# ashvardanian/StringZilla

Measured on AMD Instinct MI355X. Metric: DP cell-updates/s (GCUPS) on 1M-pair Levenshtein batch, higher is better.
Workload: dtype u32 bit-vectors (u64 results)

## Files before the change

### stringzilla_amd/csrc/hip/kernels.h

```cpp
#ifndef SZS_ROCM_KERNELS_H_
#define SZS_ROCM_KERNELS_H_

#include <stddef.h>
#include <stdint.h>

#ifdef __cplusplus
extern "C" {
#endif

typedef struct szs_string_ref_t {
    uint64_t address;
    uint32_t length;
    uint32_t index;
} szs_string_ref_t;

#define SZS_LAYOUT_SYMMETRIC 1
#define SZS_LAYOUT_TRANSPOSED 2

#define SZS_CANDIDATES_PER_WORKGROUP 256u
#define SZS_MYERS_MAX_WORDS 64u
#define SZS_MYERS_SHORT_WORDS 8u

unsigned szs_hip_levenshtein_myers_round_words(unsigned words);

// ... 171 lines not shown
    szs_knob_split_k,
    szs_knob_alphabet_k,
    szs_knob_merge_k,
    szs_knob_team_k,
    szs_knob_queues_k,
    szs_knob_roctx_k,
    szs_knob_queue_k,
    szs_knob_queue_words_k,
    szs_knob_queue_rounds_k,
    szs_knob_queue_priority_k,
    szs_knob_fused_k,
    szs_knob_tiny_k,
    szs_knob_top_k_tile_k,
    szs_knob_rerank_k,
    szs_knob_fuzzy_search_segment_k,
    szs_knob_fuzzy_scan_piece_k,
    szs_knob_count_k
};
int szs_tuning_get(int knob);


#define SZS_PLAN_VARIANTS 10u
#define SZS_PLAN_DEVICE_LONGEST 6143u
#define SZS_PLAN_STATUS_DESCENDING 1u
#define SZS_PLAN_STATUS_OVERFLOW 2u
#define SZS_PLAN_STATUS_UNSORTED 4u

typedef struct szs_side_stats_t {
    uint32_t count, longest;
    uint64_t symbols;
    uint64_t bands_systolic;
    uint64_t bands_chain;
} szs_side_stats_t;

typedef struct szs_plan_side_t {
    void const *offsets;
    uint64_t base;
    uint32_t count, wide;
    szs_string_ref_t *ascending, *descending;
    uint32_t const *lengths;
    uint64_t const *starts;
} szs_plan_side_t;

typedef struct szs_plan_expectation_t {
    uint32_t enabled;
    uint32_t query_side;
    uint32_t longest[2];
    uint32_t variant_counts[SZS_PLAN_VARIANTS];
    uint32_t sequence;
    uint64_t const *runes_needed;
    uint64_t runes_capacity;
    uint32_t const *alphabet_flags;
    uint32_t alphabet;
} szs_plan_expectation_t;

#define SZS_PLAN_RANK_SAMPLES 32u
typedef struct szs_plan_summary_t {
    uint32_t status;
    uint32_t speculation_held;
    szs_side_stats_t side[2];
    uint32_t variant_counts[2][SZS_PLAN_VARIANTS];
    uint64_t symmetric_cells;
    uint32_t sequence;
    uint32_t rank_lengths[2][SZS_PLAN_RANK_SAMPLES + 1];
} szs_plan_summary_t;
#define SZS_PLAN_TIMESTAMPS_AT 448u

int szs_hip_plan(szs_plan_side_t const *queries, szs_plan_side_t const *candidates, unsigned myers_words,
                 szs_plan_expectation_t const *expected, szs_plan_summary_t *summary,
                 uint32_t *verdicts ,
                 void *stream);

#define SZS_FUSED_MOST_STRINGS 1024u
#define SZS_FUSED_MOST_STRINGS_TWO_PASSES 16384u
#define SZS_FUSED_BINS 1024u
typedef struct szs_fused_side_report_t {
    uint32_t sequence;
    uint32_t status;
    uint32_t blank;
    uint32_t pairing;
    szs_side_stats_t stats;
    uint32_t rank_lengths[SZS_PLAN_RANK_SAMPLES + 1];
    uint32_t ticks[5];
    uint32_t padding;
    uint64_t squares;
} szs_fused_side_report_t;
typedef struct szs_fused_plan_t {
    szs_plan_side_t side[2];
    uint32_t sequence;
    uint32_t *ready;
    szs_fused_side_report_t *report;
    uint32_t *gave_up;
    uint32_t poll_budget;
    uint32_t withhold;
    uint32_t symmetric;
    uint32_t blocks_per_group;
} szs_fused_plan_t;
#define SZS_FUSED_POLL_BUDGET (1u << 18)
int szs_hip_levenshtein_myers_fused(szs_fused_plan_t const *plan, uint64_t *results, uint64_t results_row_stride, int layout,
                                    void *stream);

int szs_hip_utf8_transcode(szs_string_ref_t const *strings, uint32_t count, uint64_t const *rune_starts, uint32_t *runes,
                           uint32_t *rune_counts, uint32_t *any_multibyte, void *stream);

int szs_hip_utf8_transcode_tape(void const *data, void const *offsets, uint32_t count, int wide, void const *before_offsets,
                                uint32_t before_count, int before_wide, uint64_t capacity, uint32_t *runes, uint64_t *rune_starts,
                                uint32_t *rune_counts, uint32_t *any_multibyte, uint64_t *needed, void *alphabet_workspace, void *stream);
int szs_hip_utf8_transcode_tapes(void const *first_data, void const *first_offsets, uint32_t first_count, int first_wide,
                                 void const *second_data, void const *second_offsets, uint32_t second_count, int second_wide,
                                 uint64_t capacity, uint32_t *runes, uint64_t *rune_starts, uint32_t *rune_counts,
                                 uint32_t *any_multibyte, uint64_t *needed, void *alphabet_workspace, void *stream);

#define SZS_ALPHABET_SLOTS (1u << 16)
#define SZS_ALPHABET_MOST 4095u
#define SZS_ALPHABET_WORTH_BYTES (1u << 16)
int szs_hip_alphabet_rename(uint32_t count, uint64_t const *rune_starts, uint32_t const *rune_counts, uint32_t *runes,
                            uint32_t const *any_multibyte, void *workspace, int workspace_is_empty, uint32_t most, uint32_t *alphabet_out,
                            void *stream);
size_t szs_hip_alphabet_workspace_bytes(void);

typedef struct szs_cost_model_t {
    int16_t substitution[32 * 32];
    uint8_t byte_to_class[256];
    int32_t gap_open;
    int32_t gap_extend;
    int32_t uniform_match, uniform_mismatch;
} szs_cost_model_t;

enum {
    szs_objective_global_k = 0,
    szs_objective_local_k = 1,
    szs_objective_distance_k = 2,
    szs_objective_distance_runes_k = 3,
    szs_objective_local_saturating_k = 4
};

int szs_hip_weighted_scores(int objective, int affine, int narrow, szs_cost_model_t const *model, szs_string_ref_t const *queries,
                            uint32_t queries_count, szs_string_ref_t const *candidates, uint32_t candidates_count,
                            uint32_t longest_candidate, int64_t *results, uint64_t results_row_stride, int symmetric,
                            void *boundary, void *stream);
size_t szs_hip_weighted_boundary_bytes(int objective, int affine, int narrow, uint32_t queries_count, uint32_t candidates_count,
                                       uint32_t longest_candidate);

int szs_hip_weighted_packed_scores(int local, int affine, uint32_t classes, szs_cost_model_t const *model,
                                   szs_string_ref_t const *queries, uint32_t queries_count, szs_string_ref_t const *candidates,
                                   uint32_t candidates_count, uint32_t longest_candidate, int64_t *results,
                                   uint64_t results_row_stride, int symmetric, void *boundary, void *stream);
size_t szs_hip_weighted_packed_boundary_bytes(int local, int affine, uint32_t classes, uint32_t queries_count,
                                              uint32_t candidates_count, uint32_t longest_candidate);

unsigned szs_hip_weighted_team_shape(unsigned index);
int szs_hip_weighted_team_has_shape(unsigned shape);
uint32_t szs_hip_weighted_team_reach_limit(int objective, int wide);
int szs_hip_weighted_team_fits(unsigned shape, uint32_t classes);
unsigned szs_hip_weighted_team_candidates_per_item(unsigned shape);
int szs_hip_byte_presence(void const *data, void const *offsets, uint32_t count, int wide, uint32_t *presence, void *stream);
int szs_hip_weighted_team_scores(int objective, int affine, int wide, unsigned shape, uint32_t classes, szs_cost_model_t const *model,
                                 szs_string_ref_t const *queries, uint32_t queries_count, szs_string_ref_t const *candidates,
                                 uint32_t candidates_count, uint32_t longest_candidate, int64_t *results,
                                 uint64_t results_row_stride, int symmetric, void *workspace, void *stream);
size_t szs_hip_weighted_team_workspace_bytes(int objective, int affine, int wide, unsigned shape, uint32_t classes, uint32_t queries_count,
                                             uint32_t candidates_count, uint32_t longest_candidate);

int szs_hip_wide_scores(int objective, int affine, szs_cost_model_t const *model, szs_string_ref_t const *queries,
                        uint32_t queries_count, szs_string_ref_t const *candidates, uint32_t candidates_count,
                        uint32_t longest_query, uint32_t longest_candidate, int64_t *results, uint64_t results_row_stride,
                        int layout, void *workspace, void *stream);
// ... 37 lines not shown
```

### stringzilla_amd/csrc/hip/lev_myers.hip

```cpp
#include "myers_core.hpp"

#define SZS_PAIR_RULE_FN __host__ __device__ static inline
#include "pair_rule.h"

#include <cstdlib>

namespace szs_hip {

#ifndef SZS_MYERS_PACK_QUERIES
#define SZS_MYERS_PACK_QUERIES 1
#endif
#ifndef SZS_MYERS_PAIR_RULES
#define SZS_MYERS_PAIR_RULES 1
#endif

#ifndef SZS_MYERS_SHORT_TEXT_DWORDS
#define SZS_MYERS_SHORT_TEXT_DWORDS 2
#endif


__device__ __forceinline__ u32 bits_in_word(u32 from, u32 to, int w) {
    u32 const low = from > 32u * w ? from : 32u * w, high = to < 32u * w + 32u ? to : 32u * w + 32u;
    if (low >= high) return 0u;
    return (high - low == 32u ? ~0u : (1u << (high - low)) - 1u) << (low - 32u * w);
}

template <int words_, int text_dwords_, bool runes_, bool paired_ = false>
__device__ __forceinline__ void myers_workgroup(u32 *peq, u32 *keys, szs_string_ref_t const query,
                                                szs_string_ref_t const *__restrict__ candidates, u32 candidates_count,
                                                u32 candidate_block, u64 *__restrict__ results, u64 results_row_stride,
                                                int symmetric, szs_ref_guard_t const &guard, u32 alphabet = 0,
                                                u32 *claimed_rows = nullptr, u32 blocks_here = 1, szs_string_ref_t const second = {}) {
    static_assert(!paired_ || !runes_, "query pairs are a byte-kernel shape");
    constexpr int rows = runes_ ? rune_slots_k : byte_rows_k;
    using layout = peq_layout<words_, rows>;
    if (guard.enabled && (!ref_is_current(guard, 0, query) || (paired_ && !ref_is_current(guard, 0, second)))) {
        if (threadIdx.x == 0) *guard.stale = guard.sequence;
        return;
    }
    u32 const first_length = query.length, second_length = paired_ ? second.length : 0u;
    u32 const query_length = paired_ ? first_length + second_length : first_length;
    u32 const used_rows = paired_ ? query_length + 2u : query_length;
    u32 const pad = 32u * words_ - used_rows;
    u32 const second_row = pad + first_length + 2u;

    for (int i = threadIdx.x; i < layout::total_dwords; i += 256) peq[i] = 0;
    if constexpr (runes_) {
        if (alphabet) {
            for (u32 i = threadIdx.x; i <= alphabet; i += 256) keys[i] = 0;
            if (threadIdx.x == 0) *claimed_rows = 0;
        }
        else
            for (int i = threadIdx.x; i < rune_slots_k; i += 256) keys[i] = rune_slot_empty_k;
    }
    __syncthreads();
    if (runes_ && alphabet) {
        u32 const *pattern = reinterpret_cast<u32 const *>(query.address);
        for (u32 i = threadIdx.x; i < query_length; i += 256) {
            u32 const id = pattern[i];
            if (atomicCAS(&keys[id], 0u, ~0u) == 0u) keys[id] = atomicAdd(claimed_rows, 1u) + 1;
        }
        __syncthreads();
        for (u32 i = threadIdx.x; i < query_length; i += 256) {
            u32 const position = pad + i;
            atomicOr(&peq[layout::dword_index((int)keys[pattern[i]], (int)(position >> 5))], 1u << (position & 31));
        }
    }
    else if constexpr (runes_) {
        u32 const *pattern = reinterpret_cast<u32 const *>(query.address);
        for (u32 i = threadIdx.x; i < query_length; i += 256) {
            u32 const rune = pattern[i];
            u32 slot = rune_slot_hash(rune);
            for (;;) {
                u32 const previous = atomicCAS(&keys[slot], rune_slot_empty_k, rune);
                if (previous == rune_slot_empty_k || previous == rune) break;
                slot = (slot + 1) & (rune_slots_k - 1);
            }
            u32 const position = pad + i;
            atomicOr(&peq[layout::dword_index((int)slot, (int)(position >> 5))], 1u << (position & 31));
        }
    }
    else {
        u8 const *pattern = reinterpret_cast<u8 const *>(query.address);
        for (u32 i = threadIdx.x; i < first_length; i += 256) {
            u32 const position = pad + i;
            atomicOr(&peq[layout::dword_index(pattern[i], (int)(position >> 5))], 1u << (position & 31));
        }
        if constexpr (paired_) {
            u8 const *above = reinterpret_cast<u8 const *>(second.address);
            for (u32 i = threadIdx.x; i < second_length; i += 256) {
                u32 const position = second_row + i;
                atomicOr(&peq[layout::dword_index(above[i], (int)(position >> 5))], 1u << (position & 31));
            }
        }
    }
    __syncthreads();
    pattern_pair_t<words_> boundary;
    if constexpr (paired_) {
#pragma unroll
        for (int w = 0; w < words_; ++w) {
            boundary.separators[w] = bits_in_word(second_row - 2u, second_row, w);
            boundary.tops[w] = first_length ? bits_in_word(second_row - 3u, second_row - 2u, w) : 0u;
        }
    }

#pragma unroll 1
    for (u32 block_step = 0; block_step < blocks_here; ++block_step) {
    u32 const candidate_slot = (candidate_block - block_step) * SZS_CANDIDATES_PER_WORKGROUP + threadIdx.x;
    bool live = candidate_slot < candidates_count;
    szs_string_ref_t candidate = {0, 0, 0};
    if (live) candidate = candidates[candidate_slot];
    if (live && guard.enabled && !ref_is_current(guard, 1, candidate)) {
        *guard.stale = guard.sequence;
        live = false;
    }
    if ((symmetric & SZS_LAYOUT_SYMMETRIC) && candidate.index > query.index) live = false;
    u32 const text_length = live ? candidate.length : 0;
    u32 const longest_in_wave = wave_max_u32(text_length);
    u32 const shortest_in_wave = ~wave_max_u32(live ? ~text_length : 0u);

    u32 vp[words_], vn[words_];
#pragma unroll
    for (int w = 0; w < words_; ++w) {
        vp[w] = bits_in_word(pad, 32u * words_, w) & ~(paired_ ? boundary.separators[w] : 0u);
        vn[w] = 0;
    }

    auto take = [&](u32 symbol) {
        u32 eq[words_];
        load_match_masks<words_, rows>(peq, !runes_ ? symbol : alphabet ? keys[symbol] : find_rune_slot(keys, symbol), eq);
        if constexpr (paired_) myers_column<words_>(vp, vn, eq, boundary);
        else myers_column<words_>(vp, vn, eq);
    };

    u32 column = 0;
    if constexpr (runes_) {
        u32 const *const runes = reinterpret_cast<u32 const *>(candidate.address);
        auto quad_at = [&](u32 index) -> uint4 {
            return index < text_length ? *reinterpret_cast<uint4 const *>(runes + index) : make_uint4(0, 0, 0, 0);
        };
        if (4 <= shortest_in_wave && longest_in_wave) {
            uint4 ahead = quad_at(0);
            for (; column + 4 <= shortest_in_wave; column += 4) {
                uint4 const now = ahead;
                ahead = quad_at(column + 4);
                take(now.x), take(now.y), take(now.z), take(now.w);
            }
        }
#pragma unroll 1
        for (; column < longest_in_wave; ++column)
            if (column < text_length) take(runes[column]);
    }
    else {
        u64 const safe_address = text_length ? candidate.address : first_length || !paired_ ? query.address : second.address;
        text_stream_t text(safe_address, text_length);
        if (!text_length) text.valid_dwords = query_length ? 1 : 0;
        u32 raw_low = text.raw(0);
        u32 dword = 0;
        constexpr u32 columns_per_iteration = 4 * text_dwords_;
#ifndef SZS_MYERS_CLAMPED_READS
#define SZS_MYERS_CLAMPED_READS(TEXT_DWORDS) ((TEXT_DWORDS) == 1)
#endif
        constexpr bool clamped_reads = SZS_MYERS_CLAMPED_READS(text_dwords_);
        if (columns_per_iteration <= shortest_in_wave && longest_in_wave && query_length) {
            u32 ahead[text_dwords_];
#pragma unroll
            for (int d = 0; d < text_dwords_; ++d) ahead[d] = clamped_reads ? text.raw_clamped(1 + d) : text.raw(1 + d);
            for (; column + columns_per_iteration <= shortest_in_wave;
                 column += columns_per_iteration, dword += text_dwords_) {
                u32 symbols[text_dwords_];
                symbols[0] = text.splice(raw_low, ahead[0]);
#pragma unroll
                for (int d = 1; d < text_dwords_; ++d) symbols[d] = text.splice(ahead[d - 1], ahead[d]);
                raw_low = ahead[text_dwords_ - 1];
#pragma unroll
                for (int d = 0; d < text_dwords_; ++d)
                    ahead[d] = clamped_reads ? text.raw_clamped(dword + text_dwords_ + 1 + d)
                                             : text.raw(dword + text_dwords_ + 1 + d);
#pragma unroll
                for (int step = 0; step < 4 * text_dwords_; ++step) take((symbols[step / 4] >> (8 * (step % 4))) & 0xFFu);
            }
        }
#ifndef SZS_MYERS_MID_LOOP
#define SZS_MYERS_MID_LOOP 0
#endif
        if constexpr (SZS_MYERS_MID_LOOP && text_dwords_ > 1) {
            if (column + 4 <= shortest_in_wave && longest_in_wave && query_length) {
                u32 ahead_one = text.raw(dword + 1);
#pragma unroll 1
                for (; column + 4 <= shortest_in_wave; column += 4, ++dword) {
                    u32 const symbols = text.splice(raw_low, ahead_one);
                    raw_low = ahead_one;
                    ahead_one = text.raw(dword + 2);
#pragma unroll
                    for (int step = 0; step < 4; ++step) take((symbols >> (8 * step)) & 0xFFu);
                }
            }
        }
        if (column < longest_in_wave) {
            u32 next = text.raw(dword + 1);
#pragma unroll 1
            for (; column < longest_in_wave; column += 4, ++dword) {
                u32 const after = text.raw(dword + 2);
                u32 const symbols = text.splice(raw_low, next);
                raw_low = next, next = after;
#pragma unroll
                for (int step = 0; step < 4; ++step)
                    if (column + step < text_length) take((symbols >> (8 * step)) & 0xFFu);
            }
        }
    }

    if (live && paired_) {
        u32 first = text_length, above = text_length;
#pragma unroll
        for (int w = 0; w < words_; ++w) {
            u32 const mine = bits_in_word(pad, pad + first_length, w), theirs = bits_in_word(second_row, 32u * words_, w);
            first += (u32)__builtin_popcount(vp[w] & mine) - (u32)__builtin_popcount(vn[w] & mine);
            above += (u32)__builtin_popcount(vp[w] & theirs) - (u32)__builtin_popcount(vn[w] & theirs);
        }
        bool const transposed = (symmetric & SZS_LAYOUT_TRANSPOSED) != 0;
        u64 const one = transposed ? candidate.index : query.index, two = transposed ? candidate.index : second.index;
        u64 const one_column = transposed ? query.index : candidate.index, two_column = transposed ? second.index : candidate.index;
        results[one * results_row_stride + one_column] = first;
        results[two * results_row_stride + two_column] = above;
    }
    else if (live) {
        u32 distance = text_length;
#pragma unroll
        for (int w = 0; w < words_; ++w) distance += (u32)__builtin_popcount(vp[w]) - (u32)__builtin_popcount(vn[w]);
        bool const transposed = (symmetric & SZS_LAYOUT_TRANSPOSED) != 0;
        u64 const row = transposed ? candidate.index : query.index, column = transposed ? query.index : candidate.index;
        results[row * results_row_stride + column] = distance;
        if ((symmetric & SZS_LAYOUT_SYMMETRIC) && candidate.index != query.index)
            results[column * results_row_stride + row] = distance;
    }
    }
}

#ifndef SZS_WORK_BLOCK_MAJOR
#define SZS_WORK_BLOCK_MAJOR 1
#endif
__device__ __forceinline__ void myers_work_item(u32 candidate_blocks, u32 &query_slot, u32 &candidate_block) {
#if SZS_WORK_BLOCK_MAJOR
    u32 const queries_count = gridDim.x / candidate_blocks;
    query_slot = blockIdx.x % queries_count;
    candidate_block = candidate_blocks - 1 - blockIdx.x / queries_count;
#else
    query_slot = blockIdx.x / candidate_blocks;
    candidate_block = candidate_blocks - 1 - blockIdx.x % candidate_blocks;
#endif
}

#ifndef SZS_MYERS_LONG_WAVES
#define SZS_MYERS_LONG_WAVES 2
#endif
template <int words_>
__global__ __launch_bounds__(256, SZS_MYERS_LONG_WAVES) void levenshtein_myers_long_kernel(szs_string_ref_t const *__restrict__ queries,
                                                                      szs_string_ref_t const *__restrict__ candidates,
                                                                      u32 candidates_count, u32 candidate_blocks,
                                                                      u64 *__restrict__ results, u64 results_row_stride,
                                                                      int symmetric, szs_ref_guard_t guard) {
    __shared__ __attribute__((aligned(16))) u32 peq[peq_layout<words_>::total_dwords];
    u32 query_slot, candidate_block;
    myers_work_item(candidate_blocks, query_slot, candidate_block);
    myers_workgroup<words_, 1, false>(peq, nullptr, queries[query_slot], candidates, candidates_count, candidate_block,
                                      results, results_row_stride, symmetric, guard);
}

__device__ __forceinline__ u64 fused_offset(void const *offsets, u32 wide, u64 index) {
    return wide ? static_cast<u64 const *>(offsets)[index] : (u64) static_cast<u32 const *>(offsets)[index];
}

__device__ __forceinline__ void fused_sort_side(szs_plan_side_t const &side, u32 is_query_side, u32 choose_rule, u32 sequence, u32 *ready,
                                                u32 second_ready, u32 withhold, szs_fused_side_report_t *report, u32 *histogram ,
                                                szs_string_ref_t *staged ) {
    constexpr u32 per_thread = SZS_FUSED_MOST_STRINGS / 256;
    u32 const tid = threadIdx.x, lane = tid & 63u, wave = tid >> 6, count = side.count;
    bool const one_pass = count <= SZS_FUSED_MOST_STRINGS;
    __shared__ u32 wave_bins[4], wave_longest[4], wave_status[4];
    __shared__ unsigned long long wave_symbols[4], wave_bands_systolic[4], wave_bands_chain[4], wave_squares[4];
    __shared__ u32 rule_words[256];

    u64 const began = wall_clock64();
    for (u32 bin = tid; bin < SZS_FUSED_BINS; bin += 256) histogram[bin] = 0;
    u64 from[per_thread], to[per_thread];
#pragma unroll
    for (u32 k = 0; k < per_thread; ++k) {
        u32 const i = tid + k * 256;
        from[k] = to[k] = 0;
        if (one_pass && i < count) from[k] = fused_offset(side.offsets, side.wide, i), to[k] = fused_offset(side.offsets, side.wide, (u64)i + 1);
    }
    __syncthreads();
    u32 bins[per_thread];
    u32 status = 0, longest = 0;
    u64 symbols = 0, bands_systolic = 0, bands_chain = 0, squares = 0;
    auto count_in = [&](u64 first, u64 last) -> u32 {
        if (last < first) return status |= SZS_PLAN_STATUS_DESCENDING, ~0u;
        if (last - first > 0xFFFFFFFFull) return status |= SZS_PLAN_STATUS_OVERFLOW, ~0u;
        u32 const length = (u32)(last - first);
        symbols += length, squares += (u64)length * length, longest = length > longest ? length : longest;
        bands_systolic += length ? (length + SZS_SYSTOLIC_BAND_ROWS - 1) / SZS_SYSTOLIC_BAND_ROWS : 1;
        bands_chain += length ? (length + SZS_MYERS_CHAIN_BAND_ROWS - 1) / SZS_MYERS_CHAIN_BAND_ROWS : 1;
        u32 const bin = length < SZS_FUSED_BINS - 1 ? length : SZS_FUSED_BINS - 1;
        atomicAdd(&histogram[bin], 1u);
        return bin;
    };
    if (one_pass) {
#pragma unroll
        for (u32 k = 0; k < per_thread; ++k) {
            bins[k] = ~0u;
            if (tid + k * 256 < count) bins[k] = count_in(from[k], to[k]);
        }
    }
    else {
#pragma unroll 1
        for (u32 first = 0; first < count; first += 1024) {
            u64 some_from[4], some_to[4];
#pragma unroll
            for (u32 k = 0; k < 4; ++k) {
                u32 const i = first + tid + k * 256;
                some_from[k] = some_to[k] = 0;
                if (i < count) some_from[k] = fused_offset(side.offsets, side.wide, i), some_to[k] = fused_offset(side.offsets, side.wide, (u64)i + 1);
            }
#pragma unroll
            for (u32 k = 0; k < 4; ++k)
                if (first + tid + k * 256 < count) (void)count_in(some_from[k], some_to[k]);
        }
    }
    if (tid == 0) report->ticks[0] = (u32)began, report->ticks[1] = (u32)(wall_clock64() - began);
#pragma unroll
    for (int offset = 32; offset >= 1; offset >>= 1) {
        status |= (u32)__shfl_xor((int)status, offset, 64);
        u32 const other = (u32)__shfl_xor((int)longest, offset, 64);
        longest = other > longest ? other : longest;
    }
    if (lane == 0) wave_status[wave] = status, wave_longest[wave] = longest;
    __syncthreads();
    u32 mine[4], sum = 0;
#pragma unroll
    for (u32 k = 0; k < 4; ++k) mine[k] = histogram[4 * tid + k], sum += mine[k];
    u32 inclusive = sum;
#pragma unroll
    for (int offset = 1; offset < 64; offset <<= 1) {
        u32 const other = (u32)__shfl_up((int)inclusive, offset, 64);
        if (lane >= (u32)offset) inclusive += other;
    }
    if (lane == 63) wave_bins[wave] = inclusive;
    __syncthreads();
    status = wave_status[0] | wave_status[1] | wave_status[2] | wave_status[3];
    longest = wave_longest[0];
#pragma unroll
    for (u32 w = 1; w < 4; ++w) longest = wave_longest[w] > longest ? wave_longest[w] : longest;
    u32 running = inclusive - sum;
    for (u32 w = 0; w < wave; ++w) running += wave_bins[w];
#pragma unroll
    for (u32 k = 0; k < 4; ++k) histogram[4 * tid + k] = running, running += mine[k];
    __syncthreads();
    if (tid == 0) report->ticks[2] = (u32)(wall_clock64() - began);
    u32 const blank = status || (is_query_side && longest > 32u * SZS_MYERS_SHORT_WORDS);
    if (one_pass) {
#pragma unroll
        for (u32 k = 0; k < per_thread; ++k) {
            u32 const i = tid + k * 256;
            if (i >= count) continue;
            szs_string_ref_t ref;
            ref.address = status ? side.base : side.base + from[k], ref.length = blank ? 0u : (u32)(to[k] - from[k]), ref.index = i;
            staged[status ? i : atomicAdd(&histogram[bins[k]], 1u)] = ref;
        }
        __syncthreads();
        for (u32 position = tid; position < count; position += 256) {
            szs_string_ref_t const ref = staged[position];
            side.ascending[position] = ref, side.descending[count - 1 - position] = ref;
        }
    }
    u32 const pair_slots = szs_pair_slots(count), pair_seconds = szs_pair_seconds(count);
    bool const choosing = choose_rule && one_pass && pair_seconds;
    if (choosing) {
        constexpr u32 strides = 256 / SZS_PAIR_RULE_CANDIDATES;
        u32 me = tid;
        asm volatile("" : "+v"(me));
        u32 const rule = szs_pair_rule_candidate(me % SZS_PAIR_RULE_CANDIDATES, pair_seconds);
        u32 words = 0;
        if (me < strides * SZS_PAIR_RULE_CANDIDATES) {
#pragma unroll 4
            for (u32 slot = me / SZS_PAIR_RULE_CANDIDATES; slot < pair_seconds; slot += strides)
                words += szs_pair_slot_words(staged[count - 1 - slot].length,
                                             staged[count - 1 - szs_pair_second_rank(rule, slot, pair_slots, pair_seconds)].length);
        }
        rule_words[me] = words;
    }
    if (!one_pass) {
#pragma unroll 1
        for (u32 first = 0; first < count; first += 1024) {
            u64 some_from[4], some_to[4];
#pragma unroll
            for (u32 k = 0; k < 4; ++k) {
                u32 const i = first + tid + k * 256;
                some_from[k] = some_to[k] = 0;
                if (i < count) some_from[k] = fused_offset(side.offsets, side.wide, i), some_to[k] = fused_offset(side.offsets, side.wide, (u64)i + 1);
            }
#pragma unroll
            for (u32 k = 0; k < 4; ++k) {
                u32 const i = first + tid + k * 256;
                if (i >= count) continue;
                u32 const length = status ? 0u : (u32)(some_to[k] - some_from[k]);
                szs_string_ref_t ref;
                ref.address = status ? side.base : side.base + some_from[k], ref.length = blank ? 0u : length, ref.index = i;
                u32 const position = status ? i : atomicAdd(&histogram[length < SZS_FUSED_BINS - 1 ? length : SZS_FUSED_BINS - 1], 1u);
                side.ascending[position] = ref, side.descending[count - 1 - position] = ref;
            }
        }
    }
    __syncthreads();
    if (tid == 0) report->ticks[3] = (u32)(wall_clock64() - began);
    u32 pairing = 0;
    if (choosing && wave == 0) {
        constexpr u32 strides = 256 / SZS_PAIR_RULE_CANDIDATES;
        u32 key = ~0u;
        if (lane < SZS_PAIR_RULE_CANDIDATES) {
            u32 total = 0;
#pragma unroll
            for (u32 k = 0; k < strides; ++k) total += rule_words[lane + k * SZS_PAIR_RULE_CANDIDATES];
            key = (total << 5) | lane;
        }
#pragma unroll
        for (int offset = 16; offset >= 1; offset >>= 1) {
            u32 const other = (u32)__shfl_xor((int)key, offset, 64);
            key = other < key ? other : key;
        }
        pairing = szs_pair_rule_candidate(key & 31u, pair_seconds);
    }
    if (tid == 0) {
        if (!withhold) {
            if (is_query_side)
                __hip_atomic_store(reinterpret_cast<u64 *>(ready), ((u64)pairing << 32) | sequence, __ATOMIC_RELEASE, __HIP_MEMORY_SCOPE_AGENT);
            else
                __hip_atomic_store(ready, sequence, __ATOMIC_RELEASE, __HIP_MEMORY_SCOPE_AGENT);
            if (second_ready) __hip_atomic_store(ready + 32, sequence, __ATOMIC_RELAXED, __HIP_MEMORY_SCOPE_AGENT);
        }
        report->ticks[4] = (u32)(wall_clock64() - began);
    }
#pragma unroll
    for (int offset = 32; offset >= 1; offset >>= 1) {
        symbols += ((u64)(u32)__shfl_xor((int)(u32)(symbols >> 32), offset, 64) << 32) | (u32)__shfl_xor((int)(u32)symbols, offset, 64);
        squares += ((u64)(u32)__shfl_xor((int)(u32)(squares >> 32), offset, 64) << 32) | (u32)__shfl_xor((int)(u32)squares, offset, 64);
        bands_systolic += ((u64)(u32)__shfl_xor((int)(u32)(bands_systolic >> 32), offset, 64) << 32) | (u32)__shfl_xor((int)(u32)bands_systolic, offset, 64);
        bands_chain += ((u64)(u32)__shfl_xor((int)(u32)(bands_chain >> 32), offset, 64) << 32) | (u32)__shfl_xor((int)(u32)bands_chain, offset, 64);
    }
    if (lane == 0) wave_symbols[wave] = symbols, wave_bands_systolic[wave] = bands_systolic, wave_bands_chain[wave] = bands_chain, wave_squares[wave] = squares;
    if (tid <= SZS_PLAN_RANK_SAMPLES) {
        u32 const rank = (u32)((u64)tid * (count ? count - 1 : 0) / SZS_PLAN_RANK_SAMPLES);
        report->rank_lengths[tid] = status || !count ? 0u : one_pass ? staged[rank].length : side.ascending[rank].length;
    }
    __syncthreads();
    if (tid == 0) {
        report->status = status, report->blank = blank, report->pairing = pairing;
        report->stats.count = count, report->stats.longest = longest;
        report->stats.symbols = wave_symbols[0] + wave_symbols[1] + wave_symbols[2] + wave_symbols[3];
        report->stats.bands_systolic = wave_bands_systolic[0] + wave_bands_systolic[1] + wave_bands_systolic[2] + wave_bands_systolic[3];
        report->stats.bands_chain = wave_bands_chain[0] + wave_bands_chain[1] + wave_bands_chain[2] + wave_bands_chain[3];
        report->squares = wave_squares[0] + wave_squares[1] + wave_squares[2] + wave_squares[3];
        report->sequence = sequence;
    }
}

__device__ __forceinline__ bool fused_prologue(szs_fused_plan_t const &plan, u32 *scratch, u32 &pairing) {
    __shared__ __attribute__((aligned(16))) szs_string_ref_t staged[SZS_FUSED_MOST_STRINGS];
    for (u32 s = 0; s < (plan.symmetric ? 1u : 2u); ++s)
        if (blockIdx.x == s % gridDim.x) {
            fused_sort_side(plan.side[s], s == 0, SZS_MYERS_PAIR_RULES && SZS_MYERS_PACK_QUERIES && s == 0 && !plan.symmetric && plan.blocks_per_group == 1,
                            plan.sequence, plan.ready + 32 * s, plan.symmetric, plan.withhold, plan.report + s, scratch, staged);
            __syncthreads();
        }
    __shared__ u32 unpublished[2], published_high[2];
    if (threadIdx.x < 2) {
        u32 polls = 0;
        u64 word;
        bool published;
        while (!(published = (u32)(word = __hip_atomic_load(reinterpret_cast<u64 const *>(plan.ready + 32 * threadIdx.x), __ATOMIC_RELAXED,
                                                             __HIP_MEMORY_SCOPE_AGENT)) == plan.sequence) &&
               ++polls < plan.poll_budget)
            __builtin_amdgcn_s_sleep(8);
        unpublished[threadIdx.x] = !published, published_high[threadIdx.x] = (u32)(word >> 32);
    }
    __syncthreads();
    pairing = (u32)__builtin_amdgcn_readfirstlane((int)published_high[0]);
    if (unpublished[0] | unpublished[1]) {
        if (threadIdx.x == 0) __hip_atomic_store(plan.gave_up, plan.sequence, __ATOMIC_RELAXED, __HIP_MEMORY_SCOPE_SYSTEM);
        return false;
    }
    return true;
}

#ifndef SZS_MYERS_SHORT_WAVES
#define SZS_MYERS_SHORT_WAVES 1
#endif
constexpr u32 szs_myers_pair_words_k = SZS_PAIR_WORDS_MOST;
template <bool runes_, bool merged_, bool fused_ = false>
__device__ __forceinline__ void myers_short_body(
    szs_string_ref_t const *__restrict__ queries, szs_string_ref_t const *__restrict__ candidates, u32 candidates_count,
    u32 candidate_blocks, u64 *__restrict__ results, u64 results_row_stride, int symmetric, szs_ref_guard_t guard, u32 alphabet,
    u32 blocks_per_group, szs_fused_plan_t const *fused = nullptr) {
    constexpr bool pairs = fused_ && !merged_ && SZS_MYERS_PACK_QUERIES;
    __shared__ __attribute__((aligned(16))) u32 peq[peq_layout<pairs ? szs_myers_pair_words_k : 8, runes_ ? rune_slots_k : byte_rows_k>::total_dwords];
    u32 pairing = 0;
    if constexpr (fused_) {
        static_assert(peq_layout<8, byte_rows_k>::total_dwords >= SZS_FUSED_BINS, "the sort's histogram borrows the masks' LDS");
        if (!fused_prologue(*fused, peq, pairing)) return;
    }
    __shared__ u32 slot_keys[runes_ ? rune_slots_k : 1];
    __shared__ u32 claimed_rows;
    extern __shared__ u32 rows_of_ids[];
    u32 *const keys = runes_ && alphabet ? rows_of_ids : slot_keys;
    u32 query_slot, candidate_group;
    myers_work_item(candidate_blocks, query_slot, candidate_group);
    u32 const all_blocks = (candidates_count + SZS_CANDIDATES_PER_WORKGROUP - 1) / SZS_CANDIDATES_PER_WORKGROUP;
    u32 const first_block = merged_ ? candidate_group * blocks_per_group : candidate_group;
    u32 const blocks_here = !merged_ ? 1u : all_blocks - first_block < blocks_per_group ? all_blocks - first_block : blocks_per_group;
    u32 const candidate_block = first_block + blocks_here - 1;
    szs_string_ref_t query = queries[query_slot];
    if constexpr (fused_) {
        query.address = ((u64)(u32)__builtin_amdgcn_readfirstlane((int)(u32)(query.address >> 32)) << 32) |
                        (u32)__builtin_amdgcn_readfirstlane((int)(u32)query.address);
        query.length = (u32)__builtin_amdgcn_readfirstlane((int)query.length);
        query.index = (u32)__builtin_amdgcn_readfirstlane((int)query.index);
    }
    szs_string_ref_t second = {0, 0, 0};
    bool has_second = false;
    if constexpr (pairs) {
        if (!fused->symmetric) {
            u32 const slots = szs_pair_slots(fused->side[0].count), seconds = szs_pair_seconds(fused->side[0].count);
            if (query_slot < seconds) {
                u32 rule = pairing;
                rule = rule <= seconds ? rule : 0u;
                second = queries[szs_pair_second_rank(rule, query_slot, slots, seconds)];
                second.address = ((u64)(u32)__builtin_amdgcn_readfirstlane((int)(u32)(second.address >> 32)) << 32) |
                                 (u32)__builtin_amdgcn_readfirstlane((int)(u32)second.address);
                second.length = (u32)__builtin_amdgcn_readfirstlane((int)second.length);
                second.index = (u32)__builtin_amdgcn_readfirstlane((int)second.index);
                has_second = true;
            }
        }
    }
    u32 const words = __builtin_amdgcn_readfirstlane(query.length ? (query.length + 31u) / 32u : 1u);
    u32 const second_words = second.length ? (second.length + 31u) / 32u : 1u;
    u32 const pair_words = szs_pair_words_shared(query.length, second.length);
    if constexpr (pairs) {
        if (has_second && szs_pair_shares(pair_words, words, second_words)) {
#define SZS_MYERS_PAIR_BODY(W)                                                                                         \
    case W:                                                                                                            \
        myers_workgroup<W, SZS_MYERS_SHORT_TEXT_DWORDS, false, true>(peq, keys, query, candidates, candidates_count,   \
                                                                     candidate_block, results, results_row_stride,    \
                                                                     symmetric, guard, 0u, nullptr, 1u, second);      \
        return;
            switch (pair_words) {
                SZS_MYERS_PAIR_BODY(1)
                SZS_MYERS_PAIR_BODY(2)
                SZS_MYERS_PAIR_BODY(3)
                SZS_MYERS_PAIR_BODY(4)
                SZS_MYERS_PAIR_BODY(5)
                SZS_MYERS_PAIR_BODY(6)
                SZS_MYERS_PAIR_BODY(7)
                SZS_MYERS_PAIR_BODY(8)
                SZS_MYERS_PAIR_BODY(9)
                SZS_MYERS_PAIR_BODY(10)
            }
#undef SZS_MYERS_PAIR_BODY
        }
    }
#define SZS_MYERS_BODY(W)                                                                                              \
    case W:                                                                                                            \
        myers_workgroup<W, SZS_MYERS_SHORT_TEXT_DWORDS, runes_>(peq, keys, query, candidates, candidates_count,       \
                                                                candidate_block, results, results_row_stride,         \
                                                                symmetric, guard, alphabet, &claimed_rows, blocks_here); \
        break;
    for (u32 turn = 0; turn < (has_second ? 2u : 1u); ++turn) {
        if (turn) {
            __syncthreads();
            query = second;
        }
        switch (turn ? second_words : words) {
            SZS_MYERS_BODY(1)
            SZS_MYERS_BODY(2)
            SZS_MYERS_BODY(3)
            SZS_MYERS_BODY(4)
            SZS_MYERS_BODY(5)
            SZS_MYERS_BODY(6)
            SZS_MYERS_BODY(7)
        default:
            myers_workgroup<8, SZS_MYERS_SHORT_TEXT_DWORDS, runes_>(peq, keys, query, candidates, candidates_count,
                                                                    candidate_block, results, results_row_stride, symmetric, guard,
                                                                    alphabet, &claimed_rows, blocks_here);
            break;
        }
    }
#undef SZS_MYERS_BODY
}

template <bool runes_>
__global__ __launch_bounds__(256, SZS_MYERS_SHORT_WAVES) void levenshtein_myers_short_kernel(
    szs_string_ref_t const *__restrict__ queries, szs_string_ref_t const *__restrict__ candidates, u32 candidates_count,
    u32 candidate_blocks, u64 *__restrict__ results, u64 results_row_stride, int symmetric, szs_ref_guard_t guard, u32 alphabet,
    u32 blocks_per_group) {
    myers_short_body<runes_, false>(queries, candidates, candidates_count, candidate_blocks, results, results_row_stride, symmetric, guard,
                                    alphabet, blocks_per_group);
}

#ifndef SZS_MYERS_FUSED_WAVES
#define SZS_MYERS_FUSED_WAVES 5
#endif
template <bool merged_>
__global__ __launch_bounds__(256, SZS_MYERS_FUSED_WAVES) void levenshtein_myers_short_fused_kernel(szs_fused_plan_t plan, u32 candidate_blocks,
                                                                                                   u64 *results, u64 results_row_stride,
                                                                                                   int layout) {
    szs_ref_guard_t const none = {};
    szs_plan_side_t const &texts = plan.symmetric ? plan.side[0] : plan.side[1];
    myers_short_body<false, merged_, true>(plan.side[0].descending, texts.ascending, texts.count, candidate_blocks, results, results_row_stride,
                                           layout, none, 0u, plan.blocks_per_group, &plan);
}

template <bool runes_>
__global__ __launch_bounds__(256, SZS_MYERS_SHORT_WAVES) void levenshtein_myers_short_merged_kernel(
    szs_string_ref_t const *__restrict__ queries, szs_string_ref_t const *__restrict__ candidates, u32 candidates_count,
    u32 candidate_blocks, u64 *__restrict__ results, u64 results_row_stride, int symmetric, szs_ref_guard_t guard, u32 alphabet,
    u32 blocks_per_group) {
    myers_short_body<runes_, true>(queries, candidates, candidates_count, candidate_blocks, results, results_row_stride, symmetric, guard,
                                   alphabet, blocks_per_group);
}

constexpr int banded_widest_k = 64;
constexpr size_t banded_header_bytes_k = 256;

template <int words_>
__device__ __forceinline__ i32 myers_strips(u32 *peq, szs_string_ref_t const query, u32 strips, text_stream_t const &text,
                                            u32 text_length, u32 shortest_in_wave, u32 longest_in_wave, u32 *parked_mine) {
    using layout = peq_layout<words_>;
    constexpr u32 strip_rows = 32u * words_;
    u32 const query_length = query.length;
    u32 const pad = strips * strip_rows - query_length;
    u8 const *const pattern = reinterpret_cast<u8 const *>(query.address);
    i32 delta_sum = 0;
    for (u32 strip = 0; strip < strips; ++strip) {
        bool const first_strip = strip == 0, last_strip = strip + 1 == strips;
        __syncthreads();
        for (int i = threadIdx.x; i < layout::total_dwords; i += 256) peq[i] = 0;
        __syncthreads();
        for (u32 bit = threadIdx.x; bit < strip_rows; bit += 256) {
            u32 const position = strip * strip_rows + bit;
            if (position >= pad) atomicOr(&peq[layout::dword_index(pattern[position - pad], (int)(bit >> 5))], 1u << (bit & 31));
        }
        __syncthreads();

        u32 vp[words_], vn[words_];
#pragma unroll
        for (int w = 0; w < words_; ++w) {
            u32 const first_bit = 32u * w;
            vp[w] = !first_strip || first_bit >= pad ? ~0u : (first_bit + 32u <= pad ? 0u : (~0u << (pad - first_bit)));
            vn[w] = 0;
        }

        u32 entering = 0, leaving = 0;
        auto take = [&](u32 symbol, u32 column) {
            u32 eq[words_];
            load_match_masks<words_, byte_rows_k>(peq, symbol, eq);
            u32 const slot = 2 * (column & 15u);
            u32 const hp_in = first_strip ? 1u : (entering >> slot) & 1u;
            u32 const hn_in = first_strip ? 0u : (entering >> (slot + 1)) & 1u;
            leaving |= myers_strip_column<words_>(vp, vn, eq, hp_in, hn_in) << slot;
        };

        u32 column = 0, dword = 0;
        u32 raw_low = text.raw(0);
        if (4 <= shortest_in_wave && longest_in_wave) {
            u32 ahead = text.raw_clamped(1);
            for (; column + 4 <= shortest_in_wave; column += 4, ++dword) {
// ... 1080 lines not shown
```

### stringzilla_amd/csrc/host/ways_planned.c

```c
#include "dispatch_internal.h"

#include <stdio.h>
#include <stdlib.h>
#include <string.h>


typedef struct planned_call_t {
    szs_call_t *call;
    szs_engine_s *engine;
    szs_decision_t *remembered;
    szs_plan_side_t q_side, c_side;
    szs_pinned_words_t volatile *words;
    int use_myers, knobs_automatic, uniform_bytes;
    unsigned myers_words;
    void const *key_data[2], *key_offsets[2];
    int key_wide[2];
    szs_plan_summary_t seen;
    int have_summary;
    int runes, renumber;
    uint64_t *starts;
    uint32_t *counts, *device_flags;
    uint32_t volatile *flags;
} planned_call_t;

// ... 100 lines not shown
          remembered->tier == SZS_TIER_LANES && remembered->use_myers && !remembered->runes && !remembered->wide_cells &&
          !szs_decision_has_variant_zero(remembered) && remembered->plan.groups_count == 1 &&
          remembered->plan.groups[0].variant == SZS_MYERS_SHORT_WORDS && remembered->q_count == call->q_count && remembered->c_count == call->c_count &&
          remembered->symmetric == symmetric && remembered->key_data[0] == way->key_data[0] && remembered->key_data[1] == way->key_data[1] &&
          remembered->key_offsets[0] == way->key_offsets[0] && remembered->key_offsets[1] == way->key_offsets[1] &&
          remembered->key_wide[0] == way->key_wide[0] && remembered->key_wide[1] == way->key_wide[1]))
        return SZS_WAY_NOT_TAKEN;
    szs_decision_t const *d = remembered;
    uint32_t volatile *const stale = &way->words->stale;
    szs_ref_guard_t guard;
    memset(&guard, 0, sizeof(guard));
    guard.enabled = 1, guard.sequence = ++engine->plan_sequence, guard.stale = (uint32_t *)stale;
    for (int role = 0; role < 2; ++role) {
        szs_plan_side_t const *side = (role == 0) == (d->transposed == 0) ? &way->q_side : &way->c_side;
        if (symmetric) side = &way->q_side;
        guard.side[role].offsets = side->offsets, guard.side[role].base = side->base;
        guard.side[role].wide = side->wide, guard.side[role].count = side->count;
    }
    *stale = 0;
    sz_status_t status = szs_call_prepare(engine, d, call->device, call->stream, call->error_message);
    if (status != sz_success_k) return status;
    szs_call_phase(call, 2);
    int stalled;
    status = score(way, d, &guard, 3, d->summary.side[0].symbols, d->summary.side[1].symbols, &stalled);
    if (status != sz_success_k) return status;
    if (*stale != guard.sequence) return sz_success_k;
    remembered->refs_current = 0;
    return SZS_WAY_NOT_TAKEN;
}

static sz_status_t planned_inside_the_launch(planned_call_t *way) {
    szs_call_t *call = way->call;
    szs_engine_s *engine = way->engine;
    szs_decision_t *const remembered = way->remembered;
    int const symmetric = call->symmetric;
    int const knob = szs_tuning_get(szs_knob_fused_k);
    if (!(remembered->valid && !remembered->runes && remembered->tier == SZS_TIER_LANES && remembered->use_myers && !remembered->wide_cells &&
          !remembered->use_queue && szs_decision_is_one_launch(remembered) && remembered->plan.groups[0].variant == SZS_MYERS_SHORT_WORDS &&
          remembered->q_count == call->q_count && remembered->c_count == call->c_count && remembered->symmetric == symmetric &&
          call->q_count <= SZS_FUSED_MOST_STRINGS_TWO_PASSES && call->c_count <= SZS_FUSED_MOST_STRINGS_TWO_PASSES && way->knobs_automatic &&
          !way->uniform_bytes && knob != 0 && (!engine->fused_gave_up || knob == 2)))
        return SZS_WAY_NOT_TAKEN;
    szs_decision_t const *d = remembered;
    szs_fused_side_report_t volatile *const reports = way->words->fused_reports;
    uint32_t volatile *const gave_up = &way->words->fused_gave_up;
    szs_fused_plan_t fused;
    memset(&fused, 0, sizeof(fused));
    fused.side[0] = d->transposed ? way->c_side : way->q_side, fused.side[1] = d->transposed ? way->q_side : way->c_side;
    if (!++engine->plan_sequence) ++engine->plan_sequence;
    fused.sequence = engine->plan_sequence;
    fused.ready = szs_device_words(engine)->ready, fused.report = (szs_fused_side_report_t *)reports;
    *gave_up = 0;
    fused.gave_up = (uint32_t *)gave_up, fused.poll_budget = SZS_FUSED_POLL_BUDGET;
    if (knob == 2) fused.withhold = 1, fused.poll_budget = 64;
    sz_status_t status = szs_call_prepare(engine, d, call->device, call->stream, call->error_message);
    if (status != sz_success_k) return status;
    szs_call_phase(call, 2);
    remembered->refs_current = 0;
    hipError_t error = hipEventRecord(engine->event_start, call->stream);
    uint32_t launches = 0;
    if (error == hipSuccess) {
        error = (hipError_t)szs_hip_levenshtein_myers_fused(&fused, (uint64_t *)call->device_results, call->device_stride, d->layout, call->stream);
        launches = error == hipSuccess;
    }
    engine->last_streams = 1;
    int stalled = 0;
    engine->last_profile.planner = 4;
    status = szs_call_finish(call, d, error, sz_success_k, launches, 0, 0, 0, &stalled);
    if (status != sz_success_k) return status;
    szs_fused_side_report_t sides[2];
    memcpy(sides, (void const *)reports, sizeof(sides));
    if (*gave_up == fused.sequence) {
        engine->fused_gave_up = 1, engine->fused_zeroed = NULL;
        return SZS_WAY_NOT_TAKEN;
    }
    if (!(sides[0].sequence == fused.sequence && !sides[0].status && !sides[0].blank &&
          (symmetric || (sides[1].sequence == fused.sequence && !sides[1].status && !sides[1].blank))))
        return SZS_WAY_NOT_TAKEN;
    engine->last_pairing = sides[0].pairing;
    szs_fused_side_report_t const *const of_queries = &sides[!symmetric && d->transposed ? 1 : 0];
    szs_fused_side_report_t const *const of_candidates = symmetric ? of_queries : &sides[d->transposed ? 0 : 1];
    if (call->trace)
        for (int s = 0; s < (symmetric ? 1 : 2); ++s)
            fprintf(stderr, "fused sorter %d (10 ns ticks since it began): offsets loaded %u, positions %u, refs written %u, published %u; began %d ticks after sorter 0; pairing rule %u\n",
                    s, sides[s].ticks[1], sides[s].ticks[2], sides[s].ticks[3], sides[s].ticks[4], (int)(sides[s].ticks[0] - sides[0].ticks[0]), sides[s].pairing);
    szs_plan_summary_t seen_here = remembered->summary;
    seen_here.status = 0, seen_here.speculation_held = 1, seen_here.sequence = fused.sequence;
    seen_here.side[0] = of_queries->stats, seen_here.side[1] = of_candidates->stats;
    memcpy(seen_here.rank_lengths[0], of_queries->rank_lengths, sizeof(seen_here.rank_lengths[0]));
    memcpy(seen_here.rank_lengths[1], of_candidates->rank_lengths, sizeof(seen_here.rank_lengths[1]));
    seen_here.symmetric_cells = symmetric ? (seen_here.side[0].symbols * seen_here.side[0].symbols + of_queries->squares) / 2 : 0;
    remembered->longest[0] = seen_here.side[0].longest, remembered->longest[1] = seen_here.side[1].longest;
    complete_from_summary(way, &seen_here);
    return szs_report(sz_success_k, call->error_message, NULL);
}

static sz_status_t planned_and_speculated(planned_call_t *way) {
    szs_call_t *call = way->call;
    szs_engine_s *engine = way->engine;
    szs_decision_t *const remembered = way->remembered;
    int const symmetric = call->symmetric;
    if (!(remembered->valid && remembered->runes == way->runes && remembered->tier == SZS_TIER_LANES && remembered->q_count == call->q_count &&
          remembered->c_count == call->c_count && remembered->symmetric == symmetric && way->knobs_automatic && !way->uniform_bytes &&
          szs_decision_is_one_launch(remembered) && (remembered->use_myers || !way->runes) && (!remembered->alphabet || way->renumber)))
        return SZS_WAY_NOT_TAKEN;
    szs_decision_t const *d = remembered;
    szs_plan_expectation_t expected = {0};
    expected.enabled = 1, expected.query_side = (uint32_t)d->transposed;
    expected.longest[0] = d->longest[0], expected.longest[1] = d->longest[1];
    memcpy(expected.variant_counts, d->variant_counts, sizeof(expected.variant_counts));
    if (way->runes) {
        expected.runes_needed = (uint64_t const *)(way->device_flags + 4), expected.runes_capacity = engine->device_runes.capacity / sizeof(uint32_t);
        expected.alphabet_flags = way->device_flags, expected.alphabet = d->alphabet;
    }
    sz_status_t status = szs_call_prepare(engine, d, call->device, call->stream, call->error_message);
    if (status != sz_success_k) return status;
    szs_call_phase(call, 2);
    hipError_t error = enqueue_plan(way, &expected);
    if (error != hipSuccess) {
        (void)hipStreamSynchronize(call->stream);
        return szs_report_hip(error, call->error_message);
    }
    int stalled;
    status = score(way, d, NULL, 2, 0, 0, &stalled);
    if (status != sz_success_k) return status;
    memcpy(&way->seen, (void const *)&way->words->summary, sizeof(way->seen));
    int const reported = way->seen.sequence == expected.sequence;
    way->have_summary = reported && !way->runes;
    if (!(reported && !way->seen.status && way->seen.speculation_held))
        return SZS_WAY_NOT_TAKEN;
    complete_from_summary(way, &way->seen);
    return szs_report(sz_success_k, call->error_message, NULL);
}

static uint32_t alphabet_with_room(uint32_t distinct) {
    uint32_t const roomy = distinct + distinct / 8 + 8;
    return roomy < SZS_ALPHABET_MOST ? roomy : SZS_ALPHABET_MOST;
}

static sz_status_t planned_and_waited_for(planned_call_t *way) {
    szs_call_t *call = way->call;
    szs_engine_s *engine = way->engine;
    szs_decision_t *const remembered = way->remembered;
    hipStream_t const stream = call->stream;
    int const symmetric = call->symmetric;
    char const **error_message = call->error_message;
    szs_plan_summary_t *const seen = &way->seen;
    sz_status_t status;
    hipError_t error;
    if (!way->have_summary)
        for (int round = 0;; ++round) {
            uint64_t const capacity = engine->device_runes.capacity / sizeof(uint32_t);
            szs_plan_expectation_t none = {0};
            error = enqueue_plan(way, &none);
            hipError_t const drained = hipStreamSynchronize(stream);
            if (error == hipSuccess) error = drained;
            if (error != hipSuccess) return szs_report_hip(error, error_message);
            memcpy(seen, (void const *)&way->words->summary, sizeof(*seen));
            if (seen->sequence != none.sequence) return szs_report(sz_status_unknown_k, error_message, "The device planner did not report");
            if (!way->runes || (seen->status & (SZS_PLAN_STATUS_DESCENDING | SZS_PLAN_STATUS_OVERFLOW))) break;
            uint64_t const needed = *(uint64_t const volatile *)(way->flags + 4);
            engine->runes_needed = needed;
            if (needed <= capacity) break;
            if (round) return szs_report(sz_status_unknown_k, error_message, "The UTF-32 buffer did not settle");
            status = szs_buffer_reserve(&engine->device_runes, szs_memory_device_k, call->device, (size_t)(needed + needed / 4 + 4) * sizeof(uint32_t), error_message);
            if (status != sz_success_k) return status;
            build_sides(way);
        }
// ... 156 lines not shown
```

Measured before the change: 102,300.

## Parallelize pairing-rule scoring across waves with LDS lengths and shuffle reduction

```diff
diff --git a/stringzilla_amd/csrc/hip/kernels.h b/stringzilla_amd/csrc/hip/kernels.h
--- a/stringzilla_amd/csrc/hip/kernels.h
+++ b/stringzilla_amd/csrc/hip/kernels.h
@@ -277,7 +277,7 @@
     szs_side_stats_t stats;
     uint32_t rank_lengths[SZS_PLAN_RANK_SAMPLES + 1];
     uint32_t ticks[5];
-    uint32_t padding;
+    uint32_t first_column;
     uint64_t squares;
 } szs_fused_side_report_t;
 typedef struct szs_fused_plan_t {
diff --git a/stringzilla_amd/csrc/hip/lev_myers.hip b/stringzilla_amd/csrc/hip/lev_myers.hip
--- a/stringzilla_amd/csrc/hip/lev_myers.hip
+++ b/stringzilla_amd/csrc/hip/lev_myers.hip
@@ -30,7 +30,8 @@
                                                 szs_string_ref_t const *__restrict__ candidates, u32 candidates_count,
                                                 u32 candidate_block, u64 *__restrict__ results, u64 results_row_stride,
                                                 int symmetric, szs_ref_guard_t const &guard, u32 alphabet = 0,
-                                                u32 *claimed_rows = nullptr, u32 blocks_here = 1, szs_string_ref_t const second = {}) {
+                                                u32 *claimed_rows = nullptr, u32 blocks_here = 1, szs_string_ref_t const second = {},
+                                                u32 *first_column_stamp = nullptr) {
     static_assert(!paired_ || !runes_, "query pairs are a byte-kernel shape");
     constexpr int rows = runes_ ? rune_slots_k : byte_rows_k;
     using layout = peq_layout<words_, rows>;
@@ -157,6 +158,10 @@
         if (!text_length) text.valid_dwords = query_length ? 1 : 0;
         u32 raw_low = text.raw(0);
         u32 dword = 0;
+        if (first_column_stamp) {
+            asm volatile("" ::"v"(raw_low));
+            if (threadIdx.x == 0) *first_column_stamp = (u32)wall_clock64();
+        }
         constexpr u32 columns_per_iteration = 4 * text_dwords_;
 #ifndef SZS_MYERS_CLAMPED_READS
 #define SZS_MYERS_CLAMPED_READS(TEXT_DWORDS) ((TEXT_DWORDS) == 1)
@@ -273,16 +278,20 @@
 }
 
 __device__ __forceinline__ void fused_sort_side(szs_plan_side_t const &side, u32 is_query_side, u32 choose_rule, u32 sequence, u32 *ready,
-                                                u32 second_ready, u32 withhold, szs_fused_side_report_t *report, u32 *histogram ,
+                                                u32 second_ready, u32 withhold, szs_fused_side_report_t *report,
+                                                u32 *histogram ,
                                                 szs_string_ref_t *staged ) {
     constexpr u32 per_thread = SZS_FUSED_MOST_STRINGS / 256;
+    static_assert(SZS_FUSED_MOST_STRINGS <= SZS_FUSED_BINS, "the staged lengths take the second SZS_FUSED_BINS dwords");
     u32 const tid = threadIdx.x, lane = tid & 63u, wave = tid >> 6, count = side.count;
     bool const one_pass = count <= SZS_FUSED_MOST_STRINGS;
+    u32 *const lengths = histogram + SZS_FUSED_BINS;
     __shared__ u32 wave_bins[4], wave_longest[4], wave_status[4];
     __shared__ unsigned long long wave_symbols[4], wave_bands_systolic[4], wave_bands_chain[4], wave_squares[4];
-    __shared__ u32 rule_words[256];
+    __shared__ u32 rule_words[SZS_PAIR_RULE_CANDIDATES];
 
     u64 const began = wall_clock64();
+    if (is_query_side && tid == 0) report->first_column = 0;
     for (u32 bin = tid; bin < SZS_FUSED_BINS; bin += 256) histogram[bin] = 0;
     u64 from[per_thread], to[per_thread];
 #pragma unroll
@@ -366,7 +375,8 @@
             if (i >= count) continue;
             szs_string_ref_t ref;
             ref.address = status ? side.base : side.base + from[k], ref.length = blank ? 0u : (u32)(to[k] - from[k]), ref.index = i;
-            staged[status ? i : atomicAdd(&histogram[bins[k]], 1u)] = ref;
+            u32 const position = status ? i : atomicAdd(&histogram[bins[k]], 1u);
+            staged[position] = ref, lengths[position] = ref.length;
         }
         __syncthreads();
         for (u32 position = tid; position < count; position += 256) {
@@ -377,18 +387,41 @@
     u32 const pair_slots = szs_pair_slots(count), pair_seconds = szs_pair_seconds(count);
     bool const choosing = choose_rule && one_pass && pair_seconds;
     if (choosing) {
-        constexpr u32 strides = 256 / SZS_PAIR_RULE_CANDIDATES;
+        constexpr u32 turns = (SZS_PAIR_RULE_CANDIDATES + 3) / 4;
+        static_assert(turns <= 6 && SZS_FUSED_MOST_STRINGS / 2 * 16 < (1u << 16), "a candidate's total fits sixteen bits, a wavefront's in three registers");
         u32 me = tid;
         asm volatile("" : "+v"(me));
-        u32 const rule = szs_pair_rule_candidate(me % SZS_PAIR_RULE_CANDIDATES, pair_seconds);
-        u32 words = 0;
-        if (me < strides * SZS_PAIR_RULE_CANDIDATES) {
-#pragma unroll 4
-            for (u32 slot = me / SZS_PAIR_RULE_CANDIDATES; slot < pair_seconds; slot += strides)
-                words += szs_pair_slot_words(staged[count - 1 - slot].length,
-                                             staged[count - 1 - szs_pair_second_rank(rule, slot, pair_slots, pair_seconds)].length);
-        }
-        rule_words[me] = words;
+        u32 const my_lane = me & 63u, my_wave = (u32)__builtin_amdgcn_readfirstlane((int)(me >> 6));
+        u32 const whole_strides = pair_seconds / 64, last_slot = whole_strides * 64 + my_lane;
+        auto words_of = [&](u32 rule, u32 slot) {
+            return szs_pair_slot_words(lengths[count - 1 - slot], lengths[count - 1 - szs_pair_second_rank(rule, slot, pair_slots, pair_seconds)]);
+        };
+        u32 packed[(turns + 1) / 2] = {};
+#pragma unroll
+        for (u32 turn = 0; turn < turns; ++turn) {
+            u32 const candidate = my_wave + 4 * turn;
+            if (candidate >= SZS_PAIR_RULE_CANDIDATES) break;
+            u32 const rule = szs_pair_rule_candidate(candidate, pair_seconds);
+            u32 words = 0, stride = 0;
+#pragma unroll 1
+            for (; stride + 4 <= whole_strides; stride += 4) {
+                u32 const slot = stride * 64 + my_lane;
+                u32 const one = words_of(rule, slot), two = words_of(rule, slot + 64), three = words_of(rule, slot + 128), four = words_of(rule, slot + 192);
+                words += (one + two) + (three + four);
+            }
+#pragma unroll 1
+            for (; stride < whole_strides; ++stride) words += words_of(rule, stride * 64 + my_lane);
+            if (last_slot < pair_seconds) words += words_of(rule, last_slot);
+            packed[turn / 2] |= words << (16 * (turn % 2));
+        }
+#pragma unroll
+        for (int offset = 32; offset >= 1; offset >>= 1)
+#pragma unroll
+            for (u32 k = 0; k < (turns + 1) / 2; ++k) packed[k] += (u32)__shfl_xor((int)packed[k], offset, 64);
+        if (my_lane == 0)
+#pragma unroll
+            for (u32 turn = 0; turn < turns; ++turn)
+                if (my_wave + 4 * turn < SZS_PAIR_RULE_CANDIDATES) rule_words[my_wave + 4 * turn] = (packed[turn / 2] >> (16 * (turn % 2))) & 0xFFFFu;
     }
     if (!one_pass) {
 #pragma unroll 1
@@ -416,14 +449,8 @@
     if (tid == 0) report->ticks[3] = (u32)(wall_clock64() - began);
     u32 pairing = 0;
     if (choosing && wave == 0) {
-        constexpr u32 strides = 256 / SZS_PAIR_RULE_CANDIDATES;
         u32 key = ~0u;
-        if (lane < SZS_PAIR_RULE_CANDIDATES) {
-            u32 total = 0;
-#pragma unroll
-            for (u32 k = 0; k < strides; ++k) total += rule_words[lane + k * SZS_PAIR_RULE_CANDIDATES];
-            key = (total << 5) | lane;
-        }
+        if (lane < SZS_PAIR_RULE_CANDIDATES) key = (rule_words[lane] << 5) | lane;
 #pragma unroll
         for (int offset = 16; offset >= 1; offset >>= 1) {
             u32 const other = (u32)__shfl_xor((int)key, offset, 64);
@@ -505,9 +532,11 @@
     constexpr bool pairs = fused_ && !merged_ && SZS_MYERS_PACK_QUERIES;
     __shared__ __attribute__((aligned(16))) u32 peq[peq_layout<pairs ? szs_myers_pair_words_k : 8, runes_ ? rune_slots_k : byte_rows_k>::total_dwords];
     u32 pairing = 0;
+    u32 *first_column_stamp = nullptr;
     if constexpr (fused_) {
-        static_assert(peq_layout<8, byte_rows_k>::total_dwords >= SZS_FUSED_BINS, "the sort's histogram borrows the masks' LDS");
+        static_assert(peq_layout<8, byte_rows_k>::total_dwords >= 2 * SZS_FUSED_BINS, "the sort's histogram and staged lengths borrow the masks' LDS");
         if (!fused_prologue(*fused, peq, pairing)) return;
+        if (blockIdx.x == 2) first_column_stamp = &fused->report[0].first_column;
     }
     __shared__ u32 slot_keys[runes_ ? rune_slots_k : 1];
     __shared__ u32 claimed_rows;
@@ -552,7 +581,8 @@
     case W:                                                                                                            \
         myers_workgroup<W, SZS_MYERS_SHORT_TEXT_DWORDS, false, true>(peq, keys, query, candidates, candidates_count,   \
                                                                      candidate_block, results, results_row_stride,    \
-                                                                     symmetric, guard, 0u, nullptr, 1u, second);      \
+                                                                     symmetric, guard, 0u, nullptr, 1u, second,       \
+                                                                     first_column_stamp);                              \
         return;
             switch (pair_words) {
                 SZS_MYERS_PAIR_BODY(1)
@@ -573,7 +603,8 @@
     case W:                                                                                                            \
         myers_workgroup<W, SZS_MYERS_SHORT_TEXT_DWORDS, runes_>(peq, keys, query, candidates, candidates_count,       \
                                                                 candidate_block, results, results_row_stride,         \
-                                                                symmetric, guard, alphabet, &claimed_rows, blocks_here); \
+                                                                symmetric, guard, alphabet, &claimed_rows, blocks_here, {},  \
+                                                                turn ? nullptr : first_column_stamp);                  \
         break;
     for (u32 turn = 0; turn < (has_second ? 2u : 1u); ++turn) {
         if (turn) {
@@ -591,7 +622,8 @@
         default:
             myers_workgroup<8, SZS_MYERS_SHORT_TEXT_DWORDS, runes_>(peq, keys, query, candidates, candidates_count,
                                                                     candidate_block, results, results_row_stride, symmetric, guard,
-                                                                    alphabet, &claimed_rows, blocks_here);
+                                                                    alphabet, &claimed_rows, blocks_here, {},
+                                                                    turn ? nullptr : first_column_stamp);
             break;
         }
     }
diff --git a/stringzilla_amd/csrc/host/ways_planned.c b/stringzilla_amd/csrc/host/ways_planned.c
--- a/stringzilla_amd/csrc/host/ways_planned.c
+++ b/stringzilla_amd/csrc/host/ways_planned.c
@@ -206,8 +206,9 @@
     szs_fused_side_report_t const *const of_candidates = symmetric ? of_queries : &sides[d->transposed ? 0 : 1];
     if (call->trace)
         for (int s = 0; s < (symmetric ? 1 : 2); ++s)
-            fprintf(stderr, "fused sorter %d (10 ns ticks since it began): offsets loaded %u, positions %u, refs written %u, published %u; began %d ticks after sorter 0; pairing rule %u\n",
-                    s, sides[s].ticks[1], sides[s].ticks[2], sides[s].ticks[3], sides[s].ticks[4], (int)(sides[s].ticks[0] - sides[0].ticks[0]), sides[s].pairing);
+            fprintf(stderr, "fused sorter %d (10 ns ticks since it began): offsets loaded %u, positions %u, refs written %u, published %u; began %d ticks after sorter 0; pairing rule %u; workgroup 2 entered its first column %d ticks after sorter 0 began\n",
+                    s, sides[s].ticks[1], sides[s].ticks[2], sides[s].ticks[3], sides[s].ticks[4], (int)(sides[s].ticks[0] - sides[0].ticks[0]), sides[s].pairing,
+                    sides[0].first_column ? (int)(sides[0].first_column - sides[0].ticks[0]) : -1);
     szs_plan_summary_t seen_here = remembered->summary;
     seen_here.status = 0, seen_here.speculation_held = 1, seen_here.sequence = fused.sequence;
     seen_here.side[0] = of_queries->stats, seen_here.side[1] = of_candidates->stats;
```

Result: no change. 101,900 (-0.4%).
